# jaeyoungchoilab/Topsicle

Hardware: AMD Instinct MI355X
Metric: bases_scanned_per_sec (higher is better)
Workload: dtype u8

## Files before the change

topsicle_amd/csrc/tps_device.h:

```cpp
#pragma once
#include <stdint.h>
#include "../../include/topsicle_hip.h"

#ifdef TPS_EMU
#define TPS_DEV static inline
#define TPS_HD static inline
#define TPS_PHASE for (int tid = 0; tid < tps::NT; ++tid)
#define TPS_SYNC() ((void)0)
#define TPS_UNROLL
#define TPS_NOVEC
#define TPS_PIN_S(x) ((void)0)
#define TPS_PIN_V(x) ((void)0)
#else
#define TPS_DEV __device__ __forceinline__
#define TPS_HD __host__ __device__ inline
__device__ __forceinline__ int tps_fresh_lane() {
    int t = (int)(threadIdx.x & 63u);
    asm volatile("" : "+v"(t));
    return t;
}
#define TPS_PHASE for (int tid = tps_fresh_lane(), once_ = 1; once_; once_ = 0)
#define TPS_SYNC() do { __builtin_amdgcn_fence(__ATOMIC_SEQ_CST, "wavefront"); __builtin_amdgcn_wave_barrier(); } while (0)
#define TPS_UNROLL _Pragma("unroll")
#define TPS_NOVEC _Pragma("clang loop vectorize(disable) interleave(disable) unroll(disable)")
#define TPS_PIN_S(x) asm volatile("" : "+s"(x))
#define TPS_PIN_V(x) asm volatile("" : "+v"(x))
#endif

namespace tps {

constexpr int NT = 64;
constexpr int WPG = 4;
constexpr int WPG_MAX = 8;
constexpr uint32_t FLAG_CONFLICT = 0x80000000u;
constexpr uint32_t FLAG16 = 0x8000u;
constexpr int HIST_COPIES = 8;
constexpr int WIN_U = 4;
constexpr int COOP_MAX = 24;

typedef unsigned __int128 u128;

#ifdef TPS_EMU
TPS_DEV uint32_t alignbit(uint32_t hi, uint32_t lo, uint32_t sh) {
    return (uint32_t)(((((uint64_t)hi) << 32) | lo) >> (sh & 31));
}
TPS_DEV uint32_t udot4(uint32_t a, uint32_t b) {
    uint32_t s = 0;
    for (int i = 0; i < 4; ++i) s += ((a >> (8 * i)) & 255u) * ((b >> (8 * i)) & 255u);
    return s;
}
TPS_DEV uint32_t perm(uint32_t s0, uint32_t s1, uint32_t sel) {
    uint32_t out = 0;
    for (int i = 0; i < 4; ++i) {
        uint32_t c = (sel >> (8 * i)) & 255u, byte;
        if (c < 4) byte = (s1 >> (8 * c)) & 255u;
        else if (c < 8) byte = (s0 >> (8 * (c - 4))) & 255u;
        else byte = (c >= 13) ? 255u : 0u;
        out |= byte << (8 * i);
    }
    return out;
}
TPS_DEV int popc(uint32_t x) { return __builtin_popcount(x); }
TPS_DEV int ffs0(uint32_t x) { return __builtin_ctz(x); }
TPS_DEV uint32_t uniform(uint32_t x) { return x; }
TPS_DEV void lds_add(uint32_t* p, uint32_t v) { *p += v; }
TPS_DEV void lds_or(uint32_t* p, uint32_t v) { *p |= v; }
TPS_DEV uint32_t lds_add_ret(uint32_t* p, uint32_t v) { uint32_t o = *p; *p += v; return o; }
TPS_DEV void lds_max_u64(uint64_t* p, uint64_t v) { if (v > *p) *p = v; }
TPS_DEV void lds_max_i32(int32_t* p, int32_t v) { if (v > *p) *p = v; }
struct u32x4 { uint32_t x, y, z, w; };
struct u32x2 { uint32_t x, y; };
TPS_DEV u32x4 load16(const uint8_t* p) { return *(const u32x4*)p; }
TPS_DEV u32x2 load8(const uint8_t* p) { return *(const u32x2*)p; }
TPS_DEV uint32_t bitrev32(uint32_t x) {
    x = ((x >> 1) & 0x55555555u) | ((x & 0x55555555u) << 1);
    x = ((x >> 2) & 0x33333333u) | ((x & 0x33333333u) << 2);
    x = ((x >> 4) & 0x0F0F0F0Fu) | ((x & 0x0F0F0F0Fu) << 4);
    return __builtin_bswap32(x);
}
#else
TPS_DEV uint32_t alignbit(uint32_t hi, uint32_t lo, uint32_t sh) { return __builtin_amdgcn_alignbit(hi, lo, sh); }
TPS_DEV uint32_t udot4(uint32_t a, uint32_t b) { return __builtin_amdgcn_udot4(a, b, 0u, false); }
TPS_DEV uint32_t perm(uint32_t s0, uint32_t s1, uint32_t sel) { return __builtin_amdgcn_perm(s0, s1, sel); }
TPS_DEV int popc(uint32_t x) { return __builtin_popcount(x); }
TPS_DEV int ffs0(uint32_t x) { return __builtin_ctz(x); }
TPS_DEV uint32_t uniform(uint32_t x) { return (uint32_t)__builtin_amdgcn_readfirstlane((int)x); }
TPS_DEV void lds_add(uint32_t* p, uint32_t v) { atomicAdd(p, v); }
TPS_DEV void lds_or(uint32_t* p, uint32_t v) { atomicOr(p, v); }
TPS_DEV uint32_t lds_add_ret(uint32_t* p, uint32_t v) { return atomicAdd(p, v); }
TPS_DEV void lds_max_u64(uint64_t* p, uint64_t v) { atomicMax((unsigned long long*)p, (unsigned long long)v); }
TPS_DEV void lds_max_i32(int32_t* p, int32_t v) { atomicMax(p, v); }
typedef uint4 u32x4;
typedef uint2 u32x2;
TPS_DEV u32x4 load16(const uint8_t* p) {
    typedef unsigned int v4u __attribute__((ext_vector_type(4)));
    typedef const __attribute__((address_space(1))) v4u* gptr_t;
    const v4u t = *(gptr_t)(uintptr_t)p;
    u32x4 r;
    r.x = t.x; r.y = t.y; r.z = t.z; r.w = t.w;
    return r;
}
TPS_DEV u32x2 load8(const uint8_t* p) {
    typedef unsigned int v2u __attribute__((ext_vector_type(2)));
    typedef const __attribute__((address_space(1))) v2u* gptr_t;
    const v2u t = *(gptr_t)(uintptr_t)p;
    u32x2 r;
    r.x = t.x; r.y = t.y;
    return r;
}
TPS_DEV uint32_t bitrev32(uint32_t x) { return __builtin_bitreverse32(x); }
#endif

#ifdef TPS_EMU
TPS_DEV uint32_t lut_at(const uint32_t* lut, uint32_t v4, uint32_t amask) { return *(const uint32_t*)((const char*)lut + (v4 & amask)); }
#define lut_at_tile lut_at
#else
TPS_DEV uint32_t lut_at(const uint32_t* lut, uint32_t v4, uint32_t amask) {
    typedef const __attribute__((address_space(3))) uint32_t* lptr_t;
    const uint32_t base = (uint32_t)(uintptr_t)(lptr_t)lut;
    return *(lptr_t)(uintptr_t)((v4 & amask) | base);
}
#ifdef TPS_DIAG_NOCONF
TPS_DEV uint32_t lut_at_tile(const uint32_t* lut, uint32_t v4, uint32_t amask) {
    typedef const __attribute__((address_space(3))) uint32_t* lptr_t;
    const uint32_t base = (uint32_t)(uintptr_t)(lptr_t)lut;
    return *(lptr_t)(uintptr_t)((((v4 & amask) >> 30) | ((threadIdx.x & 63u) << 2)) | base);
}
#else
#define lut_at_tile lut_at
#endif
#endif

#ifndef TPS_WIDE16_MODE
#define TPS_WIDE16_MODE 1
#endif
#ifdef TPS_EMU
TPS_DEV uint32_t lut16_at(const uint32_t* lut, uint32_t v2, uint32_t amask1) { return *(const uint16_t*)((const char*)lut + (v2 & amask1)); }
#define lut16_at_wide lut16_at
#else
TPS_DEV uint32_t lut16_at(const uint32_t* lut, uint32_t v2, uint32_t amask1) {
    typedef const __attribute__((address_space(3))) uint16_t* lptr16_t;
    const uint32_t base = (uint32_t)(uintptr_t)(const __attribute__((address_space(3))) uint32_t*)lut;
    return *(lptr16_t)(uintptr_t)((v2 & amask1) | base);
}
TPS_DEV uint32_t lut16_at_wide(const uint32_t* lut, uint32_t v2, uint32_t amask1) {
    uint32_t h = lut16_at(lut, v2, amask1);
#if TPS_WIDE16_MODE == 1
    asm("" : "+v"(h));
#endif
    return h;
}
#endif

#ifdef TPS_EMU
TPS_DEV void g16_store(uint64_t base, uint32_t i, uint32_t v) { ((uint16_t*)(uintptr_t)base)[i] = (uint16_t)v; }
TPS_DEV uint32_t g16_load(uint64_t base, uint32_t i) { return ((const uint16_t*)(uintptr_t)base)[i]; }
#else
TPS_DEV void g16_store(uint64_t base, uint32_t i, uint32_t v) {
    typedef __attribute__((address_space(1))) uint16_t* gp_t;
    ((gp_t)(uintptr_t)base)[i] = (uint16_t)v;
}
TPS_DEV uint32_t g16_load(uint64_t base, uint32_t i) {
    typedef const __attribute__((address_space(1))) uint16_t* gp_t;
    return ((gp_t)(uintptr_t)base)[i];
}
#endif

#ifdef TPS_EMU
TPS_DEV void g32_store(uint64_t base, uint32_t i, uint32_t v) { ((uint32_t*)(uintptr_t)base)[i] = v; }
TPS_DEV uint32_t g32_load(uint64_t base, uint32_t i) { return ((const uint32_t*)(uintptr_t)base)[i]; }
#else
TPS_DEV void g32_store(uint64_t base, uint32_t i, uint32_t v) {
    typedef __attribute__((address_space(1))) uint32_t* gp_t;
    ((gp_t)(uintptr_t)base)[i] = v;
}
TPS_DEV uint32_t g32_load(uint64_t base, uint32_t i) {
    typedef const __attribute__((address_space(1))) uint32_t* gp_t;
    return ((gp_t)(uintptr_t)base)[i];
}
#endif

TPS_DEV uint32_t mulhi32(uint32_t x, uint32_t y) { return (uint32_t)(((uint64_t)x * (uint64_t)y) >> 32); }
#ifdef TPS_EMU
TPS_DEV uint32_t mul24(uint32_t x, uint32_t y) { return (x & 0xFFFFFFu) * (y & 0xFFFFFFu); }
#else
TPS_DEV uint32_t mul24(uint32_t x, uint32_t y) { return (x & 0xFFFFFFu) * (y & 0xFFFFFFu); }
#endif
#ifdef TPS_EMU
TPS_DEV uint32_t add_bytes(uint32_t v, uint32_t acc) { return acc + (v & 255u) + ((v >> 8) & 255u) + ((v >> 16) & 255u) + (v >> 24); }
#else
TPS_DEV uint32_t add_bytes(uint32_t v, uint32_t acc) { return __builtin_amdgcn_sad_u8(v, 0u, acc); }
#endif

// ... 182 lines not shown
constexpr int X_BS = 64;
constexpr int X_CD = X_BS + NT;
constexpr int X_CDEN = X_CD + 2 * NT;
constexpr int X_CB = X_CDEN + 2 * NT;
constexpr int X_R = X_CB + NT;

TPS_DEV int padded(int i, int pad_log2) { return i + (i >> pad_log2); }
#ifdef TPS_EMU
TPS_DEV uint32_t wg_exclusive_scan(uint32_t* arr, int n, uint32_t* scratch, int pad_log2 = 30) {
    (void)scratch;
    uint32_t run = 0;
    for (int i = 0; i < n; ++i) { uint32_t t = arr[padded(i, pad_log2)]; arr[padded(i, pad_log2)] = run; run += t; }
    return run;
}
#else
TPS_DEV uint32_t wg_exclusive_scan(uint32_t* arr, int n, uint32_t* scratch, int pad_log2 = 30) {
    (void)scratch;
    const int lane = (int)(threadIdx.x & 63u);
    const int per = (n + NT - 1) / NT;
    const int lo = lane * per, hi = (lo + per < n) ? lo + per : n;
    uint32_t s = 0;
    for (int i = lo; i < hi; ++i) s += arr[padded(i, pad_log2)];
    uint32_t inc = s;
    inc += (uint32_t)__builtin_amdgcn_update_dpp(0, (int)inc, 0x111, 0xf, 0xf, false);
    inc += (uint32_t)__builtin_amdgcn_update_dpp(0, (int)inc, 0x112, 0xf, 0xf, false);
    inc += (uint32_t)__builtin_amdgcn_update_dpp(0, (int)inc, 0x114, 0xf, 0xf, false);
    inc += (uint32_t)__builtin_amdgcn_update_dpp(0, (int)inc, 0x118, 0xf, 0xf, false);
    inc += (uint32_t)__builtin_amdgcn_update_dpp(0, (int)inc, 0x142, 0xa, 0xf, false);
    inc += (uint32_t)__builtin_amdgcn_update_dpp(0, (int)inc, 0x143, 0xc, 0xf, false);
    const uint32_t total = (uint32_t)__builtin_amdgcn_readlane((int)inc, 63);
    uint32_t run = inc - s;
    for (int i = lo; i < hi; ++i) { uint32_t t = arr[padded(i, pad_log2)]; arr[padded(i, pad_log2)] = run; run += t; }
    TPS_SYNC();
    return total;
}
#endif

#ifndef TPS_EMU
TPS_DEV uint32_t wave_max_u32(uint32_t v) {
    auto mx = [](uint32_t a, uint32_t b) { return a > b ? a : b; };
    v = mx(v, (uint32_t)__builtin_amdgcn_update_dpp(0, (int)v, 0x111, 0xf, 0xf, false));
    v = mx(v, (uint32_t)__builtin_amdgcn_update_dpp(0, (int)v, 0x112, 0xf, 0xf, false));
    v = mx(v, (uint32_t)__builtin_amdgcn_update_dpp(0, (int)v, 0x114, 0xf, 0xf, false));
    v = mx(v, (uint32_t)__builtin_amdgcn_update_dpp(0, (int)v, 0x118, 0xf, 0xf, false));
    v = mx(v, (uint32_t)__builtin_amdgcn_update_dpp(0, (int)v, 0x142, 0xa, 0xf, false));
    v = mx(v, (uint32_t)__builtin_amdgcn_update_dpp(0, (int)v, 0x143, 0xc, 0xf, false));
    return (uint32_t)__builtin_amdgcn_readlane((int)v, 63);
}
#endif

struct Stage {
    uint64_t q0;
    uint64_t v0;
    int32_t delta;
    int32_t nq;
    int32_t n;
    bool reverse;
};
TPS_DEV Stage stage_plan(const uint32_t* seq2_base, const uint16_t* inv_base, int64_t word_off, int64_t L, bool reverse, int64_t t, int64_t i0, int32_t n) {
    Stage st;
    st.reverse = reverse;
    st.n = n;
    const int64_t pos = reverse ? (L - 1 - t - i0) : (t + i0);
    const int64_t w = word_off + 4 * (pos >> 6);
    st.delta = reverse ? 63 - (int32_t)(pos & 63) : (int32_t)(pos & 63);
    st.q0 = (uint64_t)(uintptr_t)seq2_base + (uint64_t)w * 4u;
    st.v0 = (uint64_t)(uintptr_t)inv_base + (uint64_t)w * 2u;
    st.nq = n > 0 ? (st.delta + n + 63) >> 6 : 0;
    return st;
}
constexpr int STAGE_KMAX = 1 << 16;
TPS_DEV const uint8_t* stage_addr(const Stage& st, int c) {
    const uint8_t* base = (const uint8_t*)(uintptr_t)(st.reverse ? st.q0 - 16ull * STAGE_KMAX : st.q0);
    const uint32_t off = st.reverse ? 16u * (uint32_t)(STAGE_KMAX - c) : 16u * (uint32_t)c;
    return base + off;
}
TPS_DEV const uint8_t* stage_inv_addr(const Stage& st, int c) {
    const uint8_t* base = (const uint8_t*)(uintptr_t)(st.reverse ? st.v0 - 8ull * STAGE_KMAX : st.v0);
    const uint32_t off = st.reverse ? 8u * (uint32_t)(STAGE_KMAX - c) : 8u * (uint32_t)c;
    return base + off;
}
TPS_DEV uint32_t rev2(uint32_t x) {
    const uint32_t y = bitrev32(x);
    return ((y >> 1) & 0x55555555u) | ((y & 0x55555555u) << 1);
}
TPS_DEV u32x4 stage_orient(const Stage& st, const u32x4& v) {
    if (!st.reverse) return v;
    u32x4 r;
    r.x = rev2(v.w); r.y = rev2(v.z); r.z = rev2(v.y); r.w = rev2(v.x);
    return r;
}
TPS_DEV u32x2 stage_orient_inv(const Stage& st, const u32x2& v) {
    if (!st.reverse) return v;
    u32x2 r;
    r.x = bitrev32(v.y); r.y = bitrev32(v.x);
    return r;
}
#ifdef TPS_EMU
TPS_DEV void lds_store16(uint32_t* p, const u32x4& v) { p[0] = v.x; p[1] = v.y; p[2] = v.z; p[3] = v.w; }
TPS_DEV void lds_store8(uint32_t* p, const u32x2& v) { p[0] = v.x; p[1] = v.y; }
#else
TPS_DEV void lds_store16(uint32_t* p, const u32x4& v) { *(u32x4*)p = v; }
TPS_DEV void lds_store8(uint32_t* p, const u32x2& v) { *(u32x2*)p = v; }
#endif

TPS_DEV void stage_thread(const Stage& st, bool has_inv, uint32_t* seq2, uint16_t* val, int nqd, uint32_t* invalid_flag, int tid) {
    for (int base = tid; base < nqd; base += 4 * NT) {
        u32x4 v[4];
        u32x2 b[4];
        TPS_UNROLL
        for (int u = 0; u < 4; ++u) {
            const int c = base + u * NT;
            v[u].x = v[u].y = v[u].z = v[u].w = 0;
            b[u].x = b[u].y = 0;
            if (c < nqd && c < st.nq) {
                v[u] = load16(stage_addr(st, c));
                if (has_inv) b[u] = load8(stage_inv_addr(st, c));
            }
        }
        TPS_UNROLL
        for (int u = 0; u < 4; ++u) {
            const int c = base + u * NT;
            if (c < nqd) {
                lds_store16(seq2 + 4 * c, stage_orient(st, v[u]));
                if (has_inv) {
                    const u32x2 o = stage_orient_inv(st, b[u]);
                    if (o.x | o.y) *invalid_flag = 1u;
                    lds_store8((uint32_t*)val + 2 * c, o);
                }
            }
        }
    }
}

TPS_DEV uint32_t v_at(const uint32_t* seq2, int q) {
    int idx = q >> 4;
    return alignbit(seq2[idx + 1], seq2[idx], (uint32_t)(q & 15) * 2u);
}
TPS_DEV bool invalid_at(const uint16_t* val, int q, int k) {
    int idx = q >> 4;
    uint64_t v = (uint64_t)val[idx] | ((uint64_t)val[idx + 1] << 16) | ((uint64_t)val[idx + 2] << 32);
    return ((v >> (q & 15)) & ((1ull << k) - 1ull)) != 0;
}
constexpr int LUT_FIELDS = 32;
constexpr int LUT_M16 = 48;
constexpr int LUT_F16 = 64;
TPS_HD int pp_field(int p) { return 4 * (p & 3) + 2 * ((p >> 2) & 1) + (p >> 3); }
TPS_HD int pp_pattern(int f) { return (f >> 2) + 4 * (((f >> 1) & 1) + 2 * (f & 1)); }
TPS_HD uint32_t mask_to_fields(uint32_t m) {
    uint32_t f = 0;
    for (int p = 0; p < 16; ++p) f |= ((m >> p) & 1u) << (2 * pp_field(p));
    return f;
}
TPS_DEV uint32_t field_to_mask(uint32_t f) { return f ? 1u << pp_pattern(ffs0(f) >> 1) : 0u; }
TPS_DEV uint32_t field_to_entry(uint32_t f) { return f ? ((1u << (16 + pp_pattern(ffs0(f) >> 1))) | 1u) : 0u; }
template <int N> struct IntC { static constexpr int value = N; };
TPS_DEV uint32_t lut_mask(const uint32_t* lut, int lshift, const PatInfo& pat, uint32_t v) {
    const uint32_t code = v & pat.kmask;
    if (pat.hash_shift) {
        const uint32_t slot = (code * pat.hash_mul) >> pat.hash_shift;
        return lut[2 * slot] == code ? lut[2 * slot + 1] : 0u;
    }
    if (lshift == LUT_FIELDS) return field_to_mask(lut[code]);
    if (lshift == LUT_M16) return ((const uint16_t*)lut)[code];
    if (lshift == LUT_F16) { const uint32_t m = ((const uint16_t*)lut)[code]; return m ? 1u << pp_pattern(ffs0(m)) : 0u; }
    return lut[code] >> lshift;
}
TPS_DEV uint32_t h_at(const uint32_t* lut, int lshift, const uint32_t* seq2, const uint16_t* val, const PatInfo& pat, int q, bool any_invalid) {
    uint32_t h = lut_mask(lut, lshift, pat, v_at(seq2, q));
    if (any_invalid && h && invalid_at(val, q, pat.k)) h = 0;
    return h;
}
TPS_DEV uint32_t conflict_bits(const PatInfo& pat, uint32_t v, uint32_t h) {
    if (pat.hash_shift) return h & pat.so_mask;
    uint32_t c = 0;
    TPS_NOVEC
    for (int i = 0; i < pat.n_periods; ++i) {
        uint32_t hp = h & pat.period_pat[i];
        if (hp && (((v ^ (v >> (2 * pat.period[i]))) & pat.kmask) == 0)) c |= hp;
    }
    return c;
}

TPS_DEV void greedy_count(const uint32_t* lut, int lshift, const uint32_t* seq2, const uint16_t* val, const PatInfo& pat, int q0,
                          int npos, int bit, bool any_invalid, int& occ, int& greedy) {
    occ = 0; greedy = 0;
    int cursor = 0;
    for (int p = 0; p < npos; ++p) {
        uint32_t h = h_at(lut, lshift, seq2, val, pat, q0 + p, any_invalid);
        if ((h >> bit) & 1u) {
            ++occ;
            if (p >= cursor) { ++greedy; cursor = p + pat.k; }
        }
    }
}

template <bool PLAIN>
TPS_DEV void trc_count_thread(const ScanArgs& a, const Lds& l, const Stage& st_s, const Stage& st_e, int tid) {
    const PatInfo& pat = a.pat;
    const int side = tid >> 5, t = tid & 31;
    const int delta = side ? st_e.delta : st_s.delta;
    const uint32_t* seq2 = l.seq2 + side * a.head_dw;
    const uint16_t* val = l.val + side * a.head_dw;
    const bool inv = !PLAIN && l.misc[M_INVALID] != 0;
    const bool so = !PLAIN && pat.so_mask != 0;
    const int npos = st_s.n - pat.k + 1;
    uint32_t* hist = l.blk + (side * HIST_COPIES + (tid & (HIST_COPIES - 1))) * HIST_STRIDE;
    uint32_t cm = 0;
    for (int p0 = t * 8; p0 < npos; p0 += 32 * 8) {
        const int q0 = delta + p0, idx = q0 >> 4;
        const uint32_t sh = (uint32_t)(q0 & 15) * 2u;
        const uint32_t d0 = seq2[idx], d1 = seq2[idx + 1], d2 = seq2[idx + 2];
        const uint32_t w0 = alignbit(d1, d0, sh), w1 = alignbit(d2, d1, sh);
        uint32_t h[8], v[8];
        TPS_UNROLL
        for (int j = 0; j < 8; ++j) {
            v[j] = j ? alignbit(w1, w0, 2u * j) : w0;
            h[j] = lut_mask(l.lut, l.lshift, pat, v[j]);
        }
        TPS_UNROLL
        for (int j = 0; j < 8; ++j) {
            uint32_t hj = h[j];
            if (p0 + j >= npos) hj = 0;
            if (PLAIN) {
                if (hj) lds_add(&hist[ffs0(hj)], 1u);
            } else {
                if (hj && inv && invalid_at(val, q0 + j, pat.k)) hj = 0;
                if (hj) {
                    if (so && (hj & pat.so_mask)) cm |= conflict_bits(pat, v[j], hj);
                    do {
                        int b = ffs0(hj);
                        hj &= hj - 1;
                        lds_add(&hist[b], 1u);
                    } while (hj);
                }
            }
        }
    }
    if (!PLAIN && cm) lds_or(&l.misc[M_CMASK + side], cm);
}
TPS_DEV int min_period(const PatInfo& pat) {
    int m = pat.k;
    TPS_NOVEC
    for (int i = 0; i < pat.n_periods; ++i) m = pat.period[i] < m ? pat.period[i] : m;
    return m;
}
TPS_DEV bool trc_packed_ok(const ScanArgs& a, int npos) {
    const int nchunks = (npos + 15) >> 4, iters = (nchunks + 31) >> 5;
    const int mp = min_period(a.pat);
    int maxd = 0;
    TPS_NOVEC
    for (int i = 0; i < a.pat.n_periods; ++i) maxd = a.pat.period[i] > maxd ? a.pat.period[i] : maxd;
    return a.pat.P <= 15 && maxd <= 6 && mp >= 3 && npos <= 255 * mp && iters * ((16 + mp - 1) / mp) <= 15;
}
template <bool SO_, int FMT = 0>
TPS_DEV void trc_count_packed(const ScanArgs& a, const Lds& l, const Stage& st_s, const Stage& st_e, int tid, uint32_t* keep = nullptr) {
    const PatInfo& pat = a.pat;
    const int side = tid >> 5, t = tid & 31;
    const int delta = side ? st_e.delta : st_s.delta;
    const uint32_t* seq2 = l.seq2 + side * a.head_dw;
    constexpr bool FLD = FMT == 1, M16 = FMT == 2 || FMT == 3, F16 = FMT == 3;
    constexpr int LS = M16 ? 1 : 2;
    const uint32_t amask = pat.kmask << LS;
    const int npos = st_s.n - pat.k + 1;
    const int nchunks = (npos + 15) >> 4;
    const int k = pat.k;
    auto fieldsq = [&](uint32_t h) -> uint32_t { return FLD ? h : M16 ? mul24(h, h) : mulhi32(h, h); };
    uint32_t ne = 0, no = 0;
    uint32_t pe = 0, po = 0, te = 0, to = 0;
    uint32_t cf = 0;
    for (int c0 = 0; c0 < nchunks; c0 += 32) {
        const int c = c0 + t;
        const int bo = 2 * (delta + 16 * c) - LS;
        const int idx = bo >> 5;
        const uint32_t sh = (uint32_t)(bo & 31);
        const uint32_t d0 = seq2[idx], d1 = seq2[idx + 1], d2 = seq2[idx + 2];
        const uint32_t w0 = alignbit(d1, d0, sh), w1 = alignbit(d2, d1, sh);
        uint32_t h[16];
        TPS_UNROLL
        for (int j = 0; j < 16; ++j) {
            const uint32_t v_ = j == 0 ? w0 : alignbit(w1, w0, 2u * j);
            h[j] = M16 ? lut16_at(l.lut, v_, amask) : lut_at(l.lut, v_, amask);
        }
        const bool last_pass = 16 * (c0 + 32) + 32 > npos;
        if (last_pass) {
            int nv = npos - 16 * c;
            TPS_PIN_V(nv);
            TPS_UNROLL
            for (int j = 0; j < 16; ++j)
                if (j >= nv) h[j] = 0;
        }
        TPS_UNROLL
        for (int half = 0; half < 2; ++half) {
            uint32_t x2 = 0;
            TPS_UNROLL
            for (int j = 8 * half; j < 8 * half + 8; ++j) x2 += fieldsq(h[j]);
            ne += x2 & 0x33333333u;
            no += (x2 >> 2) & 0x33333333u;
        }
        if (SO_) {
            const uint32_t w2 = alignbit(seq2[idx + 3], d2, sh);
            const uint32_t a0 = alignbit(w1, w0, (uint32_t)LS), a1 = alignbit(w2, w1, (uint32_t)LS), a2 = w2 >> LS;
            TPS_NOVEC
            for (int pi = 0; pi < pat.n_periods; ++pi) {
                const int d = pat.period[pi];
                const uint32_t x0 = a0 ^ alignbit(a1, a0, 2u * (uint32_t)d), x1 = a1 ^ alignbit(a2, a1, 2u * (uint32_t)d);
                const uint32_t z0 = ~(x0 | (x0 >> 1)) & 0x55555555u, z1 = ~(x1 | (x1 >> 1)) & 0x55555555u;
                uint32_t r0 = z0, r1 = z1;
                TPS_NOVEC
                for (int u = 1; u < k; ++u) { r0 &= alignbit(z1, z0, 2u * (uint32_t)u); r1 &= z1 >> (2 * u); }
                uint32_t pr = r0, tr = 0, qd = 0;
                if (pat.n_periods == 1) {
                    tr = r0 & alignbit(r1, r0, 2u * (uint32_t)d);
                    qd = tr & alignbit(r1, r0, 4u * (uint32_t)d);
                    const int known = 32 - k - 2 * d;
                    if (known < 15) qd |= tr & ~((known < 0) ? 0u : ((4u << (2 * known)) - 1u));
                } else {
                    qd = pr;
                }
                if (last_pass) {
                    auto below = [&](int n) -> uint32_t { return n <= 0 ? 0u : n >= 16 ? 0xFFFFFFFFu : ((1u << (2 * n)) - 1u); };
                    pr &= below(npos - 16 * c - d);
                    tr &= below(npos - 16 * c - 2 * d);
                    if (pat.n_periods == 1) qd &= below(npos - 16 * c - 2 * d); else qd &= below(npos - 16 * c - d);
                }
#ifndef TPS_TRC_PAIRWALK
#define TPS_TRC_PAIRWALK 1
#endif
#if TPS_TRC_PAIRWALK != 0 && !defined(TPS_EMU_OLD_PAIRWALK)
                {
                    uint32_t m = pr;
                    while (m != 0u) {
                        const uint32_t j2 = (uint32_t)ffs0(m);
                        m &= m - 1u;
                        const uint32_t hj = M16 ? lut16_at(l.lut, alignbit(w1, w0, j2), amask) : lut_at(l.lut, alignbit(w1, w0, j2), amask);
                        const uint32_t f = fieldsq(hj);
                        pe += f & 0x33333333u; po += (f >> 2) & 0x33333333u;
                        if ((tr >> j2) & 1u) { te += f & 0x33333333u; to += (f >> 2) & 0x33333333u; }
                        if ((qd >> j2) & 1u) cf |= hj;
                    }
                }
#else
                if (pr != 0u) {
                    uint32_t xp[2] = {0u, 0u}, xt[2] = {0u, 0u};
                    TPS_UNROLL
                    for (int j = 0; j < 16; ++j) {
                        const uint32_t hp = h[j] & (0u - ((pr >> (2 * j)) & 1u));
                        const uint32_t ht = h[j] & (0u - ((tr >> (2 * j)) & 1u));
                        xp[j >> 3] += fieldsq(hp);
                        xt[j >> 3] += fieldsq(ht);
                        cf |= h[j] & (0u - ((qd >> (2 * j)) & 1u));
                    }
                    TPS_UNROLL
                    for (int half = 0; half < 2; ++half) {
                        pe += xp[half] & 0x33333333u; po += (xp[half] >> 2) & 0x33333333u;
                        te += xt[half] & 0x33333333u; to += (xt[half] >> 2) & 0x33333333u;
                    }
                }
#endif
            }
        }
    }
    if (SO_ && cf) {
        uint32_t cm = M16 ? cf : cf >> 16;
        if (FLD || F16) {
            cm = 0;
            while (cf) { cm |= 1u << pp_pattern(F16 ? ffs0(cf) : ffs0(cf) >> 1); cf &= cf - 1u; }
        }
        lds_or(&l.misc[M_CMASK + side], cm);
    }
    uint32_t* dst = keep ? keep : l.blk + 4 * tid;
    dst[0] = (ne & 0x0F0F0F0Fu) - (pe & 0x0F0F0F0Fu) + (te & 0x0F0F0F0Fu);
    dst[1] = ((ne >> 4) & 0x0F0F0F0Fu) - ((pe >> 4) & 0x0F0F0F0Fu) + ((te >> 4) & 0x0F0F0F0Fu);
// ... 2074 lines not shown
                int64_t d = (int64_t)n * (int64_t)run - (int64_t)tot * (int64_t)b;
                double sc = score_f64(d, (uint64_t)b * (uint64_t)(n - b));
                if (sc >= best) { second = best; best = sc; best_b = b; }
                else if (sc > second) second = sc;
            }
            run += (uint64_t)sv;
            if (++j == jump) j = 0;
        };
        int j = 0;
        if (in_regs) {
            TPS_UNROLL
            for (int i = 0; i < CHUNK_REGS; ++i)
                if (lo + i < hi) visit(lo + i, (uint32_t)S[lo + i], j);
        } else {
            for (int b = lo; b < hi; ++b) visit(b, (uint32_t)S[b], j);
        }
        uint64_t bits = 0;
        if (best >= 0.0) __builtin_memcpy(&bits, &best, 8);
        wg_max_bits(bits, (uint64_t*)&misc[M_MAXSC]);
#ifdef TPS_EMU
        keep[3 * tid] = best; keep[3 * tid + 1] = second; keep[3 * tid + 2] = (double)best_b;
#endif
    }
    TPS_SYNC();
    TPS_PHASE {
#ifdef TPS_EMU
        best = keep[3 * tid]; second = keep[3 * tid + 1]; best_b = (int)keep[3 * tid + 2];
#endif
        double m;
        __builtin_memcpy(&m, &misc[M_MAXSC], 8);
        const double thr = m * (1.0 - 1e-14);
        uint32_t near = (best >= thr && best >= 0.0 ? 1u : 0u) + (second >= thr && second >= 0.0 ? 1u : 0u);
        if (near) lds_add(&misc[M_NTIE], near);
        if (best == m && best_b >= 0) lds_max_i32((int32_t*)&misc[M_BESTB], best_b);
    }
    TPS_SYNC();
    tie = misc[M_NTIE] > 1u;
    if (tie) {
        Cand ex = binseg_exact_wg(S, n, jump, min_size, xs);
        bkp = ex.b;
        gain = ex.b < 0 ? 0.0 : gain_from((int64_t)ex.d, ex.den, n, n_patterns);
    } else {
        bkp = (int32_t)misc[M_BESTB];
        double m;
        __builtin_memcpy(&m, &misc[M_MAXSC], 8);
        gain = bkp < 0 ? 0.0 : m / (double)n / ((double)n_patterns * (double)n_patterns);
        TPS_SYNC();
    }
}

template <typename ST>
TPS_DEV void binseg_from_lc(const ScanArgs& a, const Lds& l, uint64_t lc_g, const ST* S_global, int n, uint64_t tot, int jump,
                            int min_size, int n_patterns, uint32_t* misc, uint32_t* xs, int& bkp, double& gain, bool& tie) {
    const int ncand = (n - 1) / jump;
#ifdef TPS_EMU
    double* keep = (double*)xs;
#endif
    double best = -1.0;
    int best_b = -1;
    bool amb = false;
    uint64_t bits = 0;
    const int c_min = (min_size + jump - 1) / jump > 1 ? (min_size + jump - 1) / jump : 1;
    const int c_max = (n - min_size) / jump < ncand ? (n - min_size) / jump : ncand;
    const bool exact53 = (double)n * 4294967296.0 < 9007199254740992.0 && (double)tot * (double)n < 9007199254740992.0;
    const double nf = (double)n, totf = (double)tot;
    constexpr int LCV = 16;
    const bool prefilter = !a.lc16 && lc_g && exact53 && c_max - c_min < LCV * NT;
    int nslot = c_max >= c_min ? (c_max - c_min + NT) / NT : 0;
    TPS_PIN_S(nslot);
    auto tile_sum = [&](int c) { return l.Tc[(uint32_t)(((uint64_t)(uint32_t)(c * jump) * a.tw_magic) >> 32)]; };
    float p_s1 = -1.0f, p_s2 = -1.0f, thr32 = -1.0f;
    uint32_t p_lc = 0;
    int p_c = -1;
    bool crowded = false;
#ifdef TPS_EMU
    static thread_local float ps1_keep[NT], ps2_keep[NT];
    static thread_local uint32_t plc_keep[NT];
    static thread_local int pc_keep[NT];
    float emu_m32 = 0.0f;
#endif
    if (prefilter) {
        TPS_PHASE {
            p_s1 = -1.0f; p_s2 = -1.0f; p_lc = 0; p_c = -1;
            auto group = [&](int g) {
                uint32_t lcv[4];
                TPS_UNROLL
                for (int i = 0; i < 4; ++i) {
                    const int c = c_min + tid + (4 * g + i) * NT;
                    lcv[i] = c <= c_max ? g32_load(lc_g, (uint32_t)c) : 0u;
                }
                TPS_UNROLL
                for (int i = 0; i < 4; ++i) {
                    const int c = c_min + tid + (4 * g + i) * NT;
                    const int b = c * jump;
                    const double bf = (double)b;
                    const float d32 = (float)__builtin_fma(-totf, bf, nf * (double)lcv[i]);
                    const float den32 = (float)b * (float)(n - b);
#ifdef TPS_EMU
                    float s_ = d32 * d32 * (1.0f / den32);
#else
                    float s_ = d32 * d32 * __builtin_amdgcn_rcpf(den32);
#endif
                    s_ = c <= c_max ? s_ : -1.0f;
                    const bool gt = s_ > p_s1;
                    const float lose = gt ? p_s1 : s_;
                    p_s2 = lose > p_s2 ? lose : p_s2;
                    p_lc = gt ? lcv[i] : p_lc;
                    p_c = gt ? c : p_c;
                    p_s1 = gt ? s_ : p_s1;
                }
            };
            if (nslot > 0) group(0);
            if (nslot > 4) group(1);
            if (nslot > 8) group(2);
            if (nslot > 12) group(3);
#ifdef TPS_EMU
            ps1_keep[tid] = p_s1; ps2_keep[tid] = p_s2; plc_keep[tid] = p_lc; pc_keep[tid] = p_c;
            emu_m32 = p_s1 > emu_m32 ? p_s1 : emu_m32;
#endif
        }
        float m32;
#ifdef TPS_EMU
        m32 = emu_m32;
#else
        {
            const float nn = p_s1 > 0.0f ? p_s1 : 0.0f;
            uint32_t mb;
            __builtin_memcpy(&mb, &nn, 4);
            mb = wave_max_u32(mb);
            __builtin_memcpy(&m32, &mb, 4);
        }
#endif
        thr32 = m32 * (1.0f - 1e-4f);
#ifdef TPS_EMU
        for (int t = 0; t < NT; ++t) crowded = crowded || (ps2_keep[t] >= thr32 && ps2_keep[t] >= 0.0f);
#else
        crowded = __builtin_amdgcn_ballot_w64(p_s2 >= thr32 && p_s2 >= 0.0f) != 0;
#endif
    }
    TPS_PHASE {
        double bn = -1.0, bd = 1.0;
        best_b = -1;
        amb = false;
        auto offer = [&](int c, uint32_t lc) {
            const int b = c * jump;
            const double bf = (double)b;
            double dd;
            if (exact53) dd = __builtin_fma(-totf, bf, nf * (double)lc);
            else dd = (double)((int64_t)n * (int64_t)lc - (int64_t)tot * (int64_t)b);
            const double num = dd * dd, den = bf * (nf - bf);
            const double t1 = num * bd, t2 = bn * den;
            const double diff = t1 - t2;
            const bool near = __builtin_fabs(diff) <= 1e-13 * t2;
            const bool take = diff >= 0.0;
            amb = near || (amb && !take);
            if (take) { bn = num; bd = den; best_b = b; }
        };
        if (prefilter) {
#ifdef TPS_EMU
            p_s1 = ps1_keep[tid]; p_lc = plc_keep[tid]; p_c = pc_keep[tid];
#endif
            if (p_c >= 0 && p_s1 >= thr32) offer(p_c, p_lc);
        } else if (a.lc16 && lc_g && c_max - c_min < LCV * NT) {
            uint32_t lcv[LCV];
            TPS_UNROLL
            for (int i = 0; i < LCV; ++i) {
                const int c = c_min + tid + i * NT;
                lcv[i] = c <= c_max ? g16_load(lc_g, (uint32_t)c) : 0u;
            }
            TPS_UNROLL
            for (int i = 0; i < LCV; ++i) {
                const int c = c_min + tid + i * NT;
                if (c <= c_max) offer(c, tile_sum(c) + lcv[i]);
            }
        } else {
            TPS_NOVEC
            for (int c = c_min + tid; c <= c_max; c += NT) {
                uint32_t lc;
                if (a.lc16) lc = tile_sum(c) + (lc_g ? g16_load(lc_g, (uint32_t)c) : (uint32_t)l.Lc16[c]);
                else lc = lc_g ? g32_load(lc_g, (uint32_t)c) : l.Lc[c];
                offer(c, lc);
            }
        }
        best = best_b >= 0 ? bn / bd : -1.0;
        bits = 0;
        if (best >= 0.0) __builtin_memcpy(&bits, &best, 8);
#ifdef TPS_EMU
        keep[3 * tid] = best; keep[3 * tid + 1] = amb ? 1.0 : 0.0; keep[3 * tid + 2] = (double)best_b;
#endif
// ... 177 lines not shown
            for (int w0 = 0; w0 < n_win; w0 += tw) {
                const int nw_tile = (n_win - w0) < tw ? (n_win - w0) : tw;
                const int64_t i0 = (int64_t)w0 * prm.slide;
                int64_t n_stage = n_s - i0;
                const int64_t cap = (int64_t)blk_per_tile * prm.slide + 32;
                if (n_stage > cap) n_stage = cap;
                const Stage st = stage_plan(a.seq2, a.inv, woff, L, tail == 1, prm.trimfirst, i0, (int)n_stage);
                const int blk_need = nw_tile + a.q + 1;
                const int spans = (blk_need + (1 << a.blk_log2) - 1) >> a.blk_log2;
                const int ndw = spans * a.span_dw + 8 < a.seq_dw ? spans * a.span_dw + 8 : a.seq_dw;
                TPS_PHASE { if (tid == 0) l.misc[M_INVALID] = 0; }
                TPS_SYNC();
                TPS_PHASE { stage_thread(st, has_inv, l.seq2, l.val, (ndw + 3) >> 2, &l.misc[M_INVALID], tid); }
                TPS_SYNC();
                if (w0 == 0) TPS_STAMP(5);
                TPS_PHASE {
                    for (int sp = tid; sp < spans; sp += NT) blocks_span(a, l, st.delta, sp);
                }
                TPS_SYNC();
                if (w0 == 0) TPS_STAMP(6);
                wg_exclusive_scan(l.Tot, spans, &l.misc[M_SCAN]);
                if (w0 == 0) TPS_STAMP(7);
                for (int base = 0; base < nw_tile; base += WIN_U * NT) {
                    TPS_PHASE { windows_group(a, l, st.delta, w0, nw_tile, out_base, base, tid); }
                    TPS_SYNC();
                    const uint32_t gsum = wg_exclusive_scan(l.row, WIN_U * NT, &l.misc[M_SCAN]);
                    TPS_PHASE { candidates_group(a, l, lc_gen, w0, nw_tile, base, (uint32_t)s_total, tid); }
                    s_total += gsum;
                    TPS_SYNC();
                }
                if (w0 == 0) TPS_STAMP(8);
            }
        } else {
            typedef TileGeo<SV ? SV : 1, FULL> t_;
            constexpr int PF = t_::PF;
            const TileConst tc = tile_const(a, r);
            int tw = (int)uniform((uint32_t)a.tw);
            TPS_PIN_S(tw);
            bool pp = false;
            if constexpr (RAW) pp = a.pp_d >= 0 && (SO ? a.pp_d > 0 : (a.pp_d == 0 && a.raw != nullptr));
            bool pp_expect = a.so_fast != 2;
            auto tile_stage = [&](int w0_) {
                const int64_t i0 = (int64_t)w0_ * prm.slide;
                int64_t n_stage = n_s - i0;
                int64_t cap = (int64_t)t_::BASES;
                const int64_t need = (int64_t)(tw - 1 + tc.q) * prm.slide + tc.r + 13;
                if (cap > need) cap = need;
                if (n_stage > cap) n_stage = cap;
                return stage_plan(a.seq2, a.inv, woff, L, tail == 1, prm.trimfirst, i0, (int)n_stage);
            };
            u32x4 pf[PF];
            u32x2 pv[PF];
#ifdef TPS_EMU
            u32x4 pf_keep[NT][PF];
            u32x2 pv_keep[NT][PF];
#endif
            auto pf_load = [&](const Stage& stn, int tid_) {
                TPS_UNROLL
                for (int u = 0; u < PF; ++u) {
                    const int c = tid_ + u * NT;
                    pf[u].x = pf[u].y = pf[u].z = pf[u].w = 0;
                    pv[u].x = pv[u].y = 0;
                    if (c < stn.nq) {
                        pf[u] = load16(stage_addr(stn, c));
                        if (has_inv) pv[u] = load8(stage_inv_addr(stn, c));
                    }
#ifdef TPS_EMU
                    pf_keep[tid_][u] = pf[u];
                    pv_keep[tid_][u] = pv[u];
#endif
                }
            };
            if (n_win > 0) {
                const Stage st0 = tile_stage(0);
                TPS_PHASE {
                    if (tid == 0) { l.misc[M_INVALID] = 0; l.misc[M_NTIE] = 0; }
                    pf_load(st0, tid);
                }
            }
            for (int w0 = 0, tile = 0; w0 < n_win; w0 += tw, ++tile) {
                const int nw_tile = (n_win - w0) < tw ? (n_win - w0) : tw;
                const Stage st = tile_stage(w0);
                TPS_PHASE {
                    TPS_UNROLL
                    for (int u = 0; u < PF; ++u) {
                        const int c = tid + u * NT;
#ifdef TPS_EMU
                        pf[u] = pf_keep[tid][u];
                        pv[u] = pv_keep[tid][u];
#endif
                        if (c < t_::NQ) {
                            lds_store16(l.seq2 + SEQ_LEAD + 4 * c, stage_orient(st, pf[u]));
                            if (has_inv) {
                                const u32x2 o = stage_orient_inv(st, pv[u]);
                                if (o.x | o.y) l.misc[M_INVALID] = 1u;
                                lds_store8((uint32_t*)l.val + (SEQ_LEAD >> 1) + 2 * c, o);
                            }
                        }
                    }
                    if (tid == NT - 1) {
                        u32x4 z;
                        z.x = z.y = z.z = z.w = 0;
                        lds_store16(l.seq2, z);
                        if (has_inv) { u32x2 z2; z2.x = z2.y = 0; lds_store8((uint32_t*)l.val, z2); }
                    }
                }
                TPS_SYNC();
                if (w0 + tw < n_win) {
                    const Stage stn = tile_stage(w0 + tw);
                    TPS_PHASE { pf_load(stn, tid); }
                }
                if (w0 == 0) TPS_STAMP(5);
                const int fdelta = st.delta + 16 * SEQ_LEAD;
                if constexpr (RAW) {
                    constexpr int SP = SV ? SV : 5;
                    if (pp && uniform(l.misc[M_INVALID]) == 0) {
                        if constexpr (SO) {
                            constexpr int HD = F16K ? 5 : 4, HR = (F16K ? 94 : 95) % SP;
                            const bool home = TPS_PP_RPT != 0 && a.pp_d == HD && tc.r == HR;
                            bool chained = true;
                            if (a.so_fast && !pp_expect) {
                                if (home) chained = tile_pp_s<SP, 0, HD, F16K, HR>(a, tc, l, fdelta, w0, tile, nw_tile, out_base, s_total);
                                else switch (a.pp_d) {
                                    case 2: chained = tile_pp_s<SP, 0, 2, F16K>(a, tc, l, fdelta, w0, tile, nw_tile, out_base, s_total); break;
                                    case 3: chained = tile_pp_s<SP, 0, 3, F16K>(a, tc, l, fdelta, w0, tile, nw_tile, out_base, s_total); break;
                                    case 4: chained = tile_pp_s<SP, 0, 4, F16K>(a, tc, l, fdelta, w0, tile, nw_tile, out_base, s_total); break;
                                    case 5: chained = tile_pp_s<SP, 0, 5, F16K>(a, tc, l, fdelta, w0, tile, nw_tile, out_base, s_total); break;
                                    default: chained = tile_pp_s<SP, 0, (SP < 6 ? SP : 6), F16K>(a, tc, l, fdelta, w0, tile, nw_tile, out_base, s_total); break;
                                }
                            }
                            if (!chained) { pp_expect = false; continue; }
                            const uint64_t s_before = s_total;
                            if (home) tile_pp_s<SP, HD, 0, F16K, HR>(a, tc, l, fdelta, w0, tile, nw_tile, out_base, s_total);
                            else switch (a.pp_d) {
                                case 2: tile_pp_s<SP, 2, 0, F16K>(a, tc, l, fdelta, w0, tile, nw_tile, out_base, s_total); break;
                                case 3: tile_pp_s<SP, 3, 0, F16K>(a, tc, l, fdelta, w0, tile, nw_tile, out_base, s_total); break;
                                case 4: tile_pp_s<SP, 4, 0, F16K>(a, tc, l, fdelta, w0, tile, nw_tile, out_base, s_total); break;
                                case 5: tile_pp_s<SP, 5, 0, F16K>(a, tc, l, fdelta, w0, tile, nw_tile, out_base, s_total); break;
                                default: tile_pp_s<SP, (SP < 6 ? SP : 6), 0, F16K>(a, tc, l, fdelta, w0, tile, nw_tile, out_base, s_total); break;
                            }
                            pp_expect = a.so_fast != 2 && (s_total - s_before) > (uint64_t)nw_tile * (uint64_t)(pat.P + 4);
                        } else {
                            constexpr int HR4 = 96 % SP;
                            if constexpr (PAIR && (HR4 & 1) == 0 && TPS_PP_PAIRF != 0) {
                                if (tc.r == HR4 && a.pair_n != 0) { tile_pp_s<SP, 0, 0, false, HR4, true>(a, tc, l, fdelta, w0, tile, nw_tile, out_base, s_total); continue; }
                            }
                            if (TPS_PP_RPT != 0 && tc.r == HR4) tile_pp_s<SP, 0, 0, false, HR4>(a, tc, l, fdelta, w0, tile, nw_tile, out_base, s_total);
                            else tile_pp_s<SP, 0>(a, tc, l, fdelta, w0, tile, nw_tile, out_base, s_total);
                        }
                        continue;
                    }
                    if (pp && SO) {
                        TPS_PHASE { if (tid == 0) l.misc[M_SCAN + 6] = 1u; }
                        TPS_SYNC();
                    }
                }
                if constexpr (SO && !RAW) {
                    constexpr int SP = SV ? SV : 5;
                    if (a.pp_d > 0 && uniform(l.misc[M_INVALID]) == 0) {
                        bool done = false;
#define TPS_LC_CD_RP(D_, N) case N: if constexpr (N < SP && D_ <= SP) { tile_lc_s<SP, false, (N < SP ? N : 0), false, false, (D_ <= SP ? D_ : 0)>(a, tc, l, fdelta, w0, tile, nw_tile, out_base, s_total, r); done = true; } break;
#define TPS_LC_CD(D_) case D_: switch (tc.r) { TPS_LC_CD_RP(D_, 0) TPS_LC_CD_RP(D_, 1) TPS_LC_CD_RP(D_, 2) TPS_LC_CD_RP(D_, 3) TPS_LC_CD_RP(D_, 4) TPS_LC_CD_RP(D_, 5) TPS_LC_CD_RP(D_, 6) TPS_LC_CD_RP(D_, 7) default: break; } break;
                        if (a.so_fast) {
                            if constexpr (DCLASS == 1) { switch (a.pp_d) { TPS_LC_CD(2) TPS_LC_CD(3) TPS_LC_CD(4) default: break; } }
                            else if constexpr (DCLASS == 2) { switch (a.pp_d) { TPS_LC_CD(5) TPS_LC_CD(6) default: break; } }
                            else { switch (a.pp_d) { TPS_LC_CD(2) TPS_LC_CD(3) TPS_LC_CD(4) TPS_LC_CD(5) TPS_LC_CD(6) default: break; } }
                        }
#undef TPS_LC_CD
#undef TPS_LC_CD_RP
                        if (done) continue;
                    }
                }
                constexpr int SF = SV ? SV : 1;
                constexpr bool LC = TPS_LC_TILE != 0 && !SO && !RAW;
                if (uniform(l.misc[M_INVALID]) != 0) {
                    if constexpr (LC) tile_lc_s<SF, true, -1, false, false, 0, P16K>(a, tc, l, fdelta, w0, tile, nw_tile, out_base, s_total, r);
                    else tile_fused_s<SF, SO, true, -1, false, RAW>(a, tc, l, fdelta, w0, tile, nw_tile, out_base, s_total, r);
                } else if constexpr (SO || RAW) {
                    if (tc.r == 0) tile_fused_s<SF, SO, false, 0, PAIR && !RAW, RAW>(a, tc, l, fdelta, w0, tile, nw_tile, out_base, s_total, r);
                    else tile_fused_s<SF, SO, false, -1, PAIR && !RAW, RAW>(a, tc, l, fdelta, w0, tile, nw_tile, out_base, s_total, r);
                } else {
#define TPS_TILE_RP(N) case N: if constexpr (N < SF) { if constexpr (LC) { if ((tc.q & 7) == 0) tile_lc_s<SF, false, (N < SF ? N : 0), PAIR, true, 0, P16K>(a, tc, l, fdelta, w0, tile, nw_tile, out_base, s_total, r); \
// ... 239 lines not shown
```

Before: 3785 billion.

## Hoist stage direction branch, use bfi/med3, integer prefilter score, simplify tail mask

Several micro-optimizations land together. The forward/reverse staging branch is hoisted out of the unrolled store loops via a templated direction dispatch, and rev2 now uses a single v_bfi_b32. The prefilter score uses exact 32-bit integer arithmetic with strength-reduced b and tot*b when it cannot overflow, avoiding double-precision FMA, and tracks the second maximum with fmed3. The last-pass tail masking now uses a per-lane full/partial predicate instead of a lane-varying count.

```diff
diff --git a/topsicle_amd/csrc/tps_device.h b/topsicle_amd/csrc/tps_device.h
--- a/topsicle_amd/csrc/tps_device.h
+++ b/topsicle_amd/csrc/tps_device.h
@@ -1,5 +1,6 @@
 #pragma once
 #include <stdint.h>
+#include <type_traits>
 #include "../../include/topsicle_hip.h"
 
 #ifdef TPS_EMU
@@ -72,6 +73,11 @@
 struct u32x2 { uint32_t x, y; };
 TPS_DEV u32x4 load16(const uint8_t* p) { return *(const u32x4*)p; }
 TPS_DEV u32x2 load8(const uint8_t* p) { return *(const u32x2*)p; }
+TPS_DEV float fmed3(float a, float b, float c) {
+    const float lo = a < b ? a : b, hi = a < b ? b : a;
+    const float m = hi < c ? hi : c;
+    return lo > m ? lo : m;
+}
 TPS_DEV uint32_t bitrev32(uint32_t x) {
     x = ((x >> 1) & 0x55555555u) | ((x & 0x55555555u) << 1);
     x = ((x >> 2) & 0x33333333u) | ((x & 0x33333333u) << 2);
@@ -109,6 +115,7 @@
     return r;
 }
 TPS_DEV uint32_t bitrev32(uint32_t x) { return __builtin_bitreverse32(x); }
+TPS_DEV float fmed3(float a, float b, float c) { return __builtin_amdgcn_fmed3f(a, b, c); }
 #endif
 
 #ifdef TPS_EMU
@@ -457,19 +464,45 @@
 }
 TPS_DEV uint32_t rev2(uint32_t x) {
     const uint32_t y = bitrev32(x);
-    return ((y >> 1) & 0x55555555u) | ((y & 0x55555555u) << 1);
-}
-TPS_DEV u32x4 stage_orient(const Stage& st, const u32x4& v) {
-    if (!st.reverse) return v;
+#ifdef TPS_EMU
+    return ((y >> 1) & 0x55555555u) | ((y << 1) & 0xAAAAAAAAu);
+#else
+    uint32_t r;
+    asm("v_bfi_b32 %0, %1, %2, %3" : "=v"(r) : "s"(0x55555555u), "v"(y >> 1), "v"(y << 1));
+    return r;
+#endif
+}
+TPS_DEV u32x4 rev2_quad(const u32x4& v) {
     u32x4 r;
     r.x = rev2(v.w); r.y = rev2(v.z); r.z = rev2(v.y); r.w = rev2(v.x);
     return r;
 }
-TPS_DEV u32x2 stage_orient_inv(const Stage& st, const u32x2& v) {
-    if (!st.reverse) return v;
+TPS_DEV u32x2 rev_inv(const u32x2& v) {
     u32x2 r;
     r.x = bitrev32(v.y); r.y = bitrev32(v.x);
     return r;
+}
+TPS_DEV u32x4 stage_orient(const Stage& st, const u32x4& v) {
+    if (!st.reverse) return v;
+    return rev2_quad(v);
+}
+TPS_DEV u32x2 stage_orient_inv(const Stage& st, const u32x2& v) {
+    if (!st.reverse) return v;
+    return rev_inv(v);
+}
+template <typename F>
+TPS_DEV void stage_dir(const Stage& st, F&& f) {
+    if (st.reverse) {
+        f(std::true_type{});
+#ifndef TPS_EMU
+        asm volatile(";stage_rev");
+#endif
+    } else {
+        f(std::false_type{});
+#ifndef TPS_EMU
+        asm volatile(";stage_fwd");
+#endif
+    }
 }
 #ifdef TPS_EMU
 TPS_DEV void lds_store16(uint32_t* p, const u32x4& v) { p[0] = v.x; p[1] = v.y; p[2] = v.z; p[3] = v.w; }
@@ -493,18 +526,20 @@
                 if (has_inv) b[u] = load8(stage_inv_addr(st, c));
             }
         }
-        TPS_UNROLL
-        for (int u = 0; u < 4; ++u) {
-            const int c = base + u * NT;
-            if (c < nqd) {
-                lds_store16(seq2 + 4 * c, stage_orient(st, v[u]));
-                if (has_inv) {
-                    const u32x2 o = stage_orient_inv(st, b[u]);
-                    if (o.x | o.y) *invalid_flag = 1u;
-                    lds_store8((uint32_t*)val + 2 * c, o);
-                }
-            }
-        }
+        stage_dir(st, [&](auto REV) {
+            TPS_UNROLL
+            for (int u = 0; u < 4; ++u) {
+                const int c = base + u * NT;
+                if (c < nqd) {
+                    lds_store16(seq2 + 4 * c, REV ? rev2_quad(v[u]) : v[u]);
+                    if (has_inv) {
+                        const u32x2 o = REV ? rev_inv(b[u]) : b[u];
+                        if (o.x | o.y) *invalid_flag = 1u;
+                        lds_store8((uint32_t*)val + 2 * c, o);
+                    }
+                }
+            }
+        });
     }
 }
 
@@ -659,11 +694,13 @@
         }
         const bool last_pass = 16 * (c0 + 32) + 32 > npos;
         if (last_pass) {
-            int nv = npos - 16 * c;
-            TPS_PIN_V(nv);
+            const int R = npos - 16 * c0;
+            const bool full = t < (R >> 4), part = t == (R >> 4);
             TPS_UNROLL
-            for (int j = 0; j < 16; ++j)
-                if (j >= nv) h[j] = 0;
+            for (int j = 0; j < 16; ++j) {
+                const bool keep = full || (part && j < (R & 15));
+                h[j] = keep ? h[j] : 0u;
+            }
         }
         TPS_UNROLL
         for (int half = 0; half < 2; ++half) {
@@ -2904,6 +2941,9 @@
     if (prefilter) {
         TPS_PHASE {
             p_s1 = -1.0f; p_s2 = -1.0f; p_lc = 0; p_c = -1;
+            const bool i32 = (uint64_t)n * tot < (1ull << 31);
+            const uint32_t bstep = (uint32_t)(NT * jump);
+            const uint32_t tbstep = (uint32_t)tot * bstep;
             auto group = [&](int g) {
                 uint32_t lcv[4];
                 TPS_UNROLL
@@ -2911,13 +2951,15 @@
                     const int c = c_min + tid + (4 * g + i) * NT;
                     lcv[i] = c <= c_max ? g32_load(lc_g, (uint32_t)c) : 0u;
                 }
+                uint32_t b = (uint32_t)((c_min + tid + 4 * g * NT) * jump);
+                uint32_t tb = (uint32_t)tot * b;
                 TPS_UNROLL
-                for (int i = 0; i < 4; ++i) {
+                for (int i = 0; i < 4; ++i, b += bstep, tb += tbstep) {
                     const int c = c_min + tid + (4 * g + i) * NT;
-                    const int b = c * jump;
-                    const double bf = (double)b;
-                    const float d32 = (float)__builtin_fma(-totf, bf, nf * (double)lcv[i]);
-                    const float den32 = (float)b * (float)(n - b);
+                    float d32;
+                    if (__builtin_expect(i32, 1)) d32 = (float)(int32_t)((uint32_t)n * lcv[i] - tb);
+                    else d32 = (float)__builtin_fma(-totf, (double)(int)b, nf * (double)lcv[i]);
+                    const float den32 = (float)(int)b * (float)(n - (int)b);
 #ifdef TPS_EMU
                     float s_ = d32 * d32 * (1.0f / den32);
 #else
@@ -2925,8 +2967,7 @@
 #endif
                     s_ = c <= c_max ? s_ : -1.0f;
                     const bool gt = s_ > p_s1;
-                    const float lose = gt ? p_s1 : s_;
-                    p_s2 = lose > p_s2 ? lose : p_s2;
+                    p_s2 = fmed3(p_s1, s_, p_s2);
                     p_lc = gt ? lcv[i] : p_lc;
                     p_c = gt ? c : p_c;
                     p_s1 = gt ? s_ : p_s1;
@@ -3270,22 +3311,24 @@
                 const int nw_tile = (n_win - w0) < tw ? (n_win - w0) : tw;
                 const Stage st = tile_stage(w0);
                 TPS_PHASE {
-                    TPS_UNROLL
-                    for (int u = 0; u < PF; ++u) {
-                        const int c = tid + u * NT;
-#ifdef TPS_EMU
-                        pf[u] = pf_keep[tid][u];
-                        pv[u] = pv_keep[tid][u];
-#endif
-                        if (c < t_::NQ) {
-                            lds_store16(l.seq2 + SEQ_LEAD + 4 * c, stage_orient(st, pf[u]));
-                            if (has_inv) {
-                                const u32x2 o = stage_orient_inv(st, pv[u]);
-                                if (o.x | o.y) l.misc[M_INVALID] = 1u;
-                                lds_store8((uint32_t*)l.val + (SEQ_LEAD >> 1) + 2 * c, o);
+                    stage_dir(st, [&](auto REV) {
+                        TPS_UNROLL
+                        for (int u = 0; u < PF; ++u) {
+                            const int c = tid + u * NT;
+#ifdef TPS_EMU
+                            pf[u] = pf_keep[tid][u];
+                            pv[u] = pv_keep[tid][u];
+#endif
+                            if (c < t_::NQ) {
+                                lds_store16(l.seq2 + SEQ_LEAD + 4 * c, REV ? rev2_quad(pf[u]) : pf[u]);
+                                if (has_inv) {
+                                    const u32x2 o = REV ? rev_inv(pv[u]) : pv[u];
+                                    if (o.x | o.y) l.misc[M_INVALID] = 1u;
+                                    lds_store8((uint32_t*)l.val + (SEQ_LEAD >> 1) + 2 * c, o);
+                                }
                             }
                         }
-                    }
+                    });
                     if (tid == NT - 1) {
                         u32x4 z;
                         z.x = z.y = z.z = z.w = 0;
```

Result: no change. 3798 billion (median of 6 runs) (+0.3%).
